# Rudrabha/Wav2Lip

Measured on NVIDIA H100. Metric: 96x96 face-crops/sec (B=128, T=5, mel 80x16), higher is better.
Workload: dtype f16

## Files before the change

### include/w2l.h

```cpp
#ifndef W2L_H_
#define W2L_H_

#include <stdint.h>

#ifdef __cplusplus
extern "C" {
#endif

#define W2L_ABI_VERSION 1

#define W2L_OK        0
#define W2L_EINVAL   -1
#define W2L_ENODEV   -2
#define W2L_ECUDA    -3
#define W2L_ENOMEM   -4
#define W2L_ESTATE   -5

#define W2L_NET_GENERATOR 0
#define W2L_NET_SYNCNET   1
#define W2L_NET_DISC      2
#define W2L_NET_S3FD      3

#define W2L_BLOCK_CONV_BN_RELU   0
#define W2L_BLOCK_CONVT_BN_RELU  1
// ... 75 lines not shown

int w2l_debug_layer_output(w2l_ctx* ctx, int net, int layer, float* y_dev, int* n, int* c, int* h, int* w,
                           void* stream);

int w2l_melspectrogram(w2l_ctx* ctx, const float* wav_dev, int64_t n_samples, float* mel_dev, void* stream);
int w2l_melspectrogram_host(w2l_ctx* ctx, const float* wav_host, int64_t n_samples, float* mel_host);
int64_t w2l_mel_num_frames(int64_t n_samples);

int64_t w2l_mel_num_chunks(int64_t n_frames, double fps);
int w2l_mel_chunks(w2l_ctx* ctx, const float* mel_dev, int64_t n_frames, double fps, float* chunks_dev,
                   int64_t n_chunks, void* stream);

int w2l_set_debug(w2l_ctx* ctx, int keep_all_layer_outputs);
int w2l_mel_basis_host(float* out_host);

#define W2L_KFAM_IGEMM        0
#define W2L_KFAM_PATCH        1
#define W2L_KFAM_CONVT_FUSED  2
typedef struct w2l_kernel_info {
    char    name[64];
    int32_t family;
    int32_t bn, bk, mt, head, bf16, x2, tma_epi, fold;
    int32_t m_tiles, n_tiles, grid;
} w2l_kernel_info;
int w2l_debug_kernel_table(int cap, w2l_kernel_info* out);
int w2l_debug_plan_kernels(w2l_ctx* ctx, int net, int cap, w2l_kernel_info* out);

#define W2L_TRAIN_WGRAD           1
#define W2L_TRAIN_ACCUMULATE      2
#define W2L_TRAIN_INPUT_GRAD      4
#define W2L_TRAIN_NO_STAT_UPDATE  8
int w2l_train_bind(w2l_ctx* ctx, int net, int n_tensors, const char* const* names, void* const* value_ptrs,
                   void* const* grad_ptrs, const int64_t* numels);

int w2l_train_forward(w2l_ctx* ctx, int net, const float* in0_dev, const float* in1_dev, float* out0_dev, float* out1_dev,
                      int B, int T, int flags, void* stream);

int w2l_train_backward(w2l_ctx* ctx, int net, const float* d0_dev, const float* d1_dev, float* dinput_dev, int flags,
                       void* stream);

int w2l_adam_step(w2l_ctx* ctx, int net, float lr, float beta1, float beta2, float eps, void* stream);

int w2l_wav2lip_train_step(w2l_ctx* ctx, const float* indiv_mels_dev, const float* x_dev, const float* mel_dev,
                           const float* gt_dev, int B, int T, float syncnet_wt, float lr, float* losses_dev, void* stream);
int w2l_train_last_output(w2l_ctx* ctx, float* out_dev, int64_t n, void* stream);
double w2l_train_flops(w2l_ctx* ctx, int net);
// ... 56 lines not shown
```

### wav2lip_b200/_lib.py

```python
from __future__ import annotations

import ctypes as C
import os
from typing import Optional

HERE = os.path.dirname(os.path.abspath(__file__))

W2L_OK, W2L_EINVAL, W2L_ENODEV, W2L_ECUDA, W2L_ENOMEM, W2L_ESTATE = 0, -1, -2, -3, -4, -5
NET_GENERATOR, NET_SYNCNET, NET_DISC, NET_S3FD = 0, 1, 2, 3
BLOCK_CONV_BN_RELU, BLOCK_CONVT_BN_RELU, BLOCK_CONV_LRELU, BLOCK_CONV_PLAIN, BLOCK_CONV_RELU = 0, 1, 2, 3, 4
PREC_F16, PREC_BF16, PREC_F32X = 0, 1, 2
TRAIN_WGRAD, TRAIN_ACCUMULATE, TRAIN_INPUT_GRAD, TRAIN_NO_STAT_UPDATE = 1, 2, 4, 8

EXPORTS = [
    "w2l_abi_version", "w2l_last_error", "w2l_net_num_layers", "w2l_net_layer_info",
    "w2l_create", "w2l_destroy", "w2l_load_weights",
    "w2l_generator_forward", "w2l_generator_forward_host", "w2l_generator_forward_u8", "w2l_generator_forward_u8_host",
    "w2l_generator_submit_host", "w2l_generator_submit_u8_host", "w2l_host_wait",
    "w2l_syncnet_forward", "w2l_syncnet_forward_frames", "w2l_cosine_bce_loss", "w2l_l1_loss", "w2l_disc_forward",
    "w2l_conv_block_forward", "w2l_debug_layer_output",
    "w2l_melspectrogram", "w2l_melspectrogram_host", "w2l_mel_num_frames", "w2l_mel_num_chunks", "w2l_mel_chunks",
    "w2l_set_debug", "w2l_mel_basis_host", "w2l_launch_count", "w2l_device_bytes", "w2l_profile_plan",
    "w2l_f16_overflow",
    "w2l_crop_resize_u8", "w2l_paste_u8", "w2l_lipsync_frames_u8", "w2l_s3fd_out_dims", "w2l_s3fd_forward",
    "w2l_train_bind", "w2l_train_forward", "w2l_train_backward", "w2l_adam_step", "w2l_wav2lip_train_step",
    "w2l_train_last_output", "w2l_train_flops", "w2l_comm_unique_id", "w2l_comm_init", "w2l_conv_block_train", "w2l_train_profile",
    "w2l_debug_kernel_table", "w2l_debug_plan_kernels", "w2l_debug_train_blocks", "w2l_debug_train_tensor",
]
KFAM_IGEMM, KFAM_PATCH, KFAM_CONVT_FUSED = 0, 1, 2
WG_PLAIN, WG_STRIDED, WG_TRANSPOSED, WG_SWAP, WG_FOLDED = 0, 1, 2, 3, 4
TAPE_X, TAPE_Z, TAPE_Y, TAPE_DY, TAPE_DZ, TAPE_DU, TAPE_DX, TAPE_DX_ADD, TAPE_STATS = range(9)


class W2LError(RuntimeError):
    pass


class LayerInfo(C.Structure):
    _fields_ = [("name", C.c_char * 64), ("kind", C.c_int32), ("cin", C.c_int32), ("cout", C.c_int32),
                ("kh", C.c_int32), ("kw", C.c_int32), ("sh", C.c_int32), ("sw", C.c_int32),
                ("ph", C.c_int32), ("pw", C.c_int32), ("out_pad", C.c_int32), ("residual", C.c_int32), ("cout_real", C.c_int32)]


class KernelInfo(C.Structure):
    _fields_ = [("name", C.c_char * 64), ("family", C.c_int32), ("bn", C.c_int32), ("bk", C.c_int32), ("mt", C.c_int32),
                ("head", C.c_int32), ("bf16", C.c_int32), ("x2", C.c_int32), ("tma_epi", C.c_int32), ("fold", C.c_int32),
                ("m_tiles", C.c_int32), ("n_tiles", C.c_int32), ("grid", C.c_int32)]

    def as_dict(self) -> dict:
        d = {f: getattr(self, f) for f, _ in self._fields_}
        d["name"] = self.name.decode()
        return d


class TrainBlockInfo(C.Structure):
    _fields_ = ([("name", C.c_char * 64)]
                + [(f, C.c_int32) for f in (
                    "layer", "kind", "cin", "cout", "kh", "kw", "sh", "sw", "ph", "pw", "out_pad", "residual",
                    "n", "h_in", "w_in", "h_out", "w_out", "lane", "has_dx", "has_dx_add", "has_du", "has_wgrad",
                    "wg_bn", "wg_form", "wg_ntaps", "wg_tg", "wg_ngroups", "wg_p", "wg_bw", "wg_bh", "wg_bnb",
                    "wg_chunks", "wg_m_tiles", "wg_n_tiles", "wg_splits", "wg_grid", "n_fwd", "n_dgrad")]
                + [("fwd", KernelInfo * 4), ("dgrad", KernelInfo * 4)])

    def as_dict(self) -> dict:
        d = {f: getattr(self, f) for f, _ in self._fields_ if f not in ("name", "fwd", "dgrad")}
        d["name"] = self.name.decode()
        d["fwd"] = [self.fwd[i].as_dict() for i in range(self.n_fwd)]
        d["dgrad"] = [self.dgrad[i].as_dict() for i in range(self.n_dgrad)]
        return d

# ... 209 lines not shown
```

### wav2lip_b200/csrc/conv_igemm.cuh

```cuda
#pragma once

#include <cuda.h>
#include <cuda_bf16.h>
#include <cuda_fp16.h>
#include <stdint.h>

#include "wgmma.cuh"

namespace w2l {

constexpr int kTileM = 128;
constexpr int kMaxTaps = 49;
constexpr int kMaxSteps = 3 * kMaxTaps;
constexpr int kSmemExtra = 2048;
constexpr int kSmemMax = 227 * 1024;
constexpr int kSmemBudget = kSmemMax - kSmemExtra - 2 * xbuf_bytes<32>();

enum : int { ACT_NONE = 0, ACT_RELU = 1, ACT_LRELU = 2 };

struct EpiParams {
    int Wout, Hout, N;
    int act;
    int out_f32;
    void* out;
    long long out_sn, out_sy, out_sx;
    const void* res;
    long long res_sn, res_sy, res_sx;
    const float* scale;
    const float* shift;
    const float* head_w;
    const float* head_b;
    int x2;
    int out_lo_off, res_lo_off;
    float* head_out;
    unsigned char* head_out_u8;
    int head_B, head_T;
};

struct alignas(64) ConvParams {
    CUtensorMap tmA;
    CUtensorMap tmB;
    CUtensorMap tmO;
    CUtensorMap tmR;
    int tma_epi;
    unsigned epi_box_bytes;
    int tiles_x, tiles_y, tiles_n, n_tiles;
    int bw, bh, bn;
    int sx, sy;
    int ntaps, kc_per_tap;
    unsigned stage_tx_bytes;
    EpiParams ep;
    int a_lo_off;
    signed char dx[kMaxSteps];
    signed char dy[kMaxSteps];
    unsigned char a_lo[kMaxSteps];
    unsigned char b_slab[kMaxSteps];
};

__device__ __forceinline__ uint32_t smem_u32(const void* p) {
    return static_cast<uint32_t>(__cvta_generic_to_shared(p));
}
__device__ __forceinline__ void mbar_init(uint32_t bar, uint32_t count) {
    asm volatile("mbarrier.init.shared::cta.b64 [%0], %1;" ::"r"(bar), "r"(count) : "memory");
}
__device__ __forceinline__ void mbar_arrive(uint32_t bar) {
    asm volatile("mbarrier.arrive.shared::cta.b64 _, [%0];" ::"r"(bar) : "memory");
// ... 10 lines not shown
        "@p bra W2L_DONE_%=;\n\t"
        "bra W2L_WAIT_%=;\n\t"
        "W2L_DONE_%=:\n\t"
        "}" ::"r"(bar), "r"(parity)
        : "memory");
}
__device__ __forceinline__ void fence_barrier_init() {
    asm volatile("fence.mbarrier_init.release.cluster;" ::: "memory");
}
__device__ __forceinline__ void tma_prefetch_desc(const void* desc) {
    asm volatile("prefetch.tensormap [%0];" ::"l"(reinterpret_cast<uint64_t>(desc)) : "memory");
}
__device__ __forceinline__ void tma_load_4d(uint32_t dst, const void* desc, uint32_t bar, int c0, int c1, int c2,
                                            int c3) {
    asm volatile(
        "cp.async.bulk.tensor.4d.shared::cluster.global.mbarrier::complete_tx::bytes [%0], [%1, {%3, %4, %5, %6}], [%2];"
        ::"r"(dst), "l"(reinterpret_cast<uint64_t>(desc)), "r"(bar), "r"(c0), "r"(c1), "r"(c2), "r"(c3)
        : "memory");
}
__device__ __forceinline__ void tma_load_3d(uint32_t dst, const void* desc, uint32_t bar, int c0, int c1, int c2) {
    asm volatile(
        "cp.async.bulk.tensor.3d.shared::cluster.global.mbarrier::complete_tx::bytes [%0], [%1, {%3, %4, %5}], [%2];"
        ::"r"(dst), "l"(reinterpret_cast<uint64_t>(desc)), "r"(bar), "r"(c0), "r"(c1), "r"(c2)
        : "memory");
}
__device__ __forceinline__ void pdl_launch_dependents() { asm volatile("griddepcontrol.launch_dependents;" ::: "memory"); }
__device__ __forceinline__ void pdl_wait() { asm volatile("griddepcontrol.wait;" ::: "memory"); }

template <int BK>
__device__ __forceinline__ uint64_t make_kmajor_desc(uint32_t saddr) {
    return wg_desc(saddr, 16, 8 * BK * 2, BK * 2);
}

template <int BN, int BK, bool kBF16>
__device__ __forceinline__ void wg_mma_tile(float (&acc)[2][BN / 2], uint32_t a, uint32_t sbo_a, uint32_t b, bool accumulate) {
#pragma unroll
    for (int k = 0; k < BK / 16; ++k) {
        const uint64_t bd = make_kmajor_desc<BK>(b + 32u * k);
        const uint32_t on = (accumulate || k > 0) ? 1u : 0u;
        wgmma_m64k16<BN, kBF16>(acc[0], wg_desc(a + 32u * k, 16, sbo_a, BK * 2), bd, on, 0);
        wgmma_m64k16<BN, kBF16>(acc[1], wg_desc(a + 8u * sbo_a + 32u * k, 16, sbo_a, BK * 2), bd, on, 0);
    }
}

template <int BN, int BK, int MT = 1>
struct ConvCfg {
// ... 152 lines not shown
    static_assert(!kHead || BN == 32, "fused head expects the 32-channel output block");
    static_assert(MT == 1 || MT == 2, "one or two M tiles per unit");

    extern __shared__ uint8_t smem_raw[];
    const uint32_t smem_raw_u32 = smem_u32(smem_raw);
    const uint32_t smem_base = (smem_raw_u32 + 1023u) & ~1023u;
    const uint32_t grp_base = smem_base + Cfg::kRingBytes;
    const uint32_t bar_base = grp_base + 2 * Cfg::kGrpBytes;
    auto full_bar = [&](int s) { return bar_base + 8u * s; };
    auto empty_bar = [&](int s) { return bar_base + 8u * (kStages + s); };
    auto res_bar = [&](int g) { return bar_base + 8u * (2 * kStages + g); };

    const int warp = threadIdx.x >> 5;
    const int lane = threadIdx.x & 31;

    if (warp == 0 && lane == 0) {
        tma_prefetch_desc(&p.tmA);
        tma_prefetch_desc(&p.tmB);
        if (p.tma_epi) {
            tma_prefetch_desc(&p.tmO);
            tma_prefetch_desc(&p.tmR);
        }
    }
    if (warp == 1 && lane == 0) {
        for (int s = 0; s < kStages; ++s) {
            mbar_init(full_bar(s), 1);
            mbar_init(empty_bar(s), 4 * MT);
        }
        for (int g = 0; g < 2; ++g) mbar_init(res_bar(g), 1);
        fence_barrier_init();
    }
    __syncthreads();
    pdl_wait();

    const int m_tiles = p.tiles_x * p.tiles_y * p.tiles_n;
    const int m_units = (m_tiles + MT - 1) / MT;
    const int total_tiles = m_units * p.n_tiles;
    const int k_steps = p.ntaps * p.kc_per_tap;

    if (warp < 4) {
        setmaxnreg_dec<kProducerRegs>();
        if (warp == 0 && lane == 0) {
            int stage = 0;
            uint32_t phase = 0;
            for (int tile = blockIdx.x; tile < total_tiles; tile += gridDim.x) {
                const int nt = tile % p.n_tiles;
                const int mu = tile / p.n_tiles;
                int x_in0[MT], y_in0[MT], n0[MT];
#pragma unroll
                for (int mt = 0; mt < MT; ++mt) {
                    const int m = mu * MT + mt;
                    const int tx = m % p.tiles_x;
                    const int ty = (m / p.tiles_x) % p.tiles_y;
                    const int tn = m / (p.tiles_x * p.tiles_y);
                    x_in0[mt] = tx * p.bw * p.sx;
                    y_in0[mt] = ty * p.bh * p.sy;
                    n0[mt] = tn * p.bn;
                }
                for (int t = 0; t < p.ntaps; ++t) {
                    for (int kc = 0; kc < p.kc_per_tap; ++kc) {
                        mbar_wait(empty_bar(stage), phase ^ 1u);
                        const uint32_t a_dst = smem_base + stage * Cfg::kStageBytes;
                        const uint32_t b_dst = a_dst + Cfg::kABytes;
                        mbar_arrive_expect_tx(full_bar(stage), p.stage_tx_bytes);
#pragma unroll
                        for (int mt = 0; mt < MT; ++mt)
                            tma_load_4d(a_dst + mt * Cfg::kATile, &p.tmA, full_bar(stage), kc * BK + (p.a_lo[t] ? p.a_lo_off : 0),
                                        x_in0[mt] + p.dx[t], y_in0[mt] + p.dy[t], n0[mt]);
                        tma_load_3d(b_dst, &p.tmB, full_bar(stage), kc * BK, nt * BN, p.b_slab[t]);
                        if (++stage == kStages) { stage = 0; phase ^= 1u; }
                    }
                }
            }
        }
    } else {
        setmaxnreg_inc<kConsumerRegs>();
        const int g = (warp - 4) >> 2;
        const int q = (warp - 4) & 3;
        const int mt = MT == 2 ? g : 0;
        constexpr int kItStride = MT == 2 ? 1 : 2;
        const int it0 = MT == 2 ? 0 : g;
        const int rows_valid = p.bw * p.bh * p.bn;
        const uint32_t bar_id = 1 + g;
        const uint32_t my_turn = 3 + g, their_turn = 3 + (g ^ 1);
        const uint32_t grp = grp_base + g * Cfg::kGrpBytes;
        float acc[2][BN / 2];
        auto mainloop = [&](int s0, bool hand_off) {
            int stage = s0 % kStages;
            uint32_t phase = static_cast<uint32_t>(s0 / kStages) & 1u;
            int prev = -1;
            for (int ks = 0; ks < k_steps; ++ks) {
                mbar_wait(full_bar(stage), phase);
                const uint32_t a_addr = smem_base + stage * Cfg::kStageBytes + mt * Cfg::kATile;
                wg_fence();
                wg_mma_tile<BN, BK, kBF16>(acc, a_addr, 8 * BK * 2, smem_base + stage * Cfg::kStageBytes + Cfg::kABytes, ks > 0);
                wg_commit();
                wg_wait<1>();
                if (prev >= 0 && lane == 0) mbar_arrive(empty_bar(prev));
                prev = stage;
                if (++stage == kStages) { stage = 0; phase ^= 1u; }
            }
            if (hand_off) named_bar_arrive(their_turn, 256);
            wg_wait<0>();
            wg_fence_regs<BN / 2>(acc[0]);
            wg_fence_regs<BN / 2>(acc[1]);
            if (prev >= 0 && lane == 0) mbar_arrive(empty_bar(prev));
        };
        auto for_each_tile = [&](auto&& epilogue) {
            for (int it = it0;; it += kItStride) {
                const int tile = blockIdx.x + it * static_cast<int>(gridDim.x);
                if (tile >= total_tiles) break;
                if (MT == 1 && it > 0) named_bar_sync(my_turn, 256);
                mainloop(it * k_steps, MT == 1 && tile + static_cast<int>(gridDim.x) < total_tiles);
                epilogue(tile, tile + kItStride * static_cast<int>(gridDim.x) < total_tiles);
            }
        };
        auto tile_origin = [&](int tile_, int* nt_, int* x0_, int* y0_, int* n0_) {
            *nt_ = tile_ % p.n_tiles;
            const int m_ = (tile_ / p.n_tiles) * MT + mt;
            *x0_ = (m_ % p.tiles_x) * p.bw;
            *y0_ = ((m_ / p.tiles_x) % p.tiles_y) * p.bh;
            *n0_ = (m_ / (p.tiles_x * p.tiles_y)) * p.bn;
        };
        if (!kHead && p.tma_epi) {
            constexpr int EW = Cfg::kEW;
            constexpr int kPasses = Cfg::kPasses;
            constexpr uint32_t kRowB = EW * 2;
            constexpr uint32_t kSwz = (kRowB == 128) ? 7u : (kRowB == 64) ? 3u : 1u;
            const bool leader = (q == 0 && lane == 0);
            const bool has_res = p.ep.res != nullptr;
            const EpiParams& e = p.ep;
            auto fetch_res = [&](int tile_) {
                int nt_, x0_, y0_, n0_;
                tile_origin(tile_, &nt_, &x0_, &y0_, &n0_);
                mbar_arrive_expect_tx(res_bar(g), kPasses * p.epi_box_bytes);
#pragma unroll
                for (int ps = 0; ps < kPasses; ++ps)
                    tma_load_4d(grp + ps * Cfg::kBoxBytes, &p.tmR, res_bar(g), nt_ * BN + ps * EW, x0_, y0_, n0_);
            };
            if (has_res && leader) {
                const int first = blockIdx.x + it0 * static_cast<int>(gridDim.x);
                if (first < total_tiles) fetch_res(first);
            }
            uint32_t rphase = 0;
            for_each_tile([&](int tile, bool more) {
                int nt, x0, y0, n0;
                tile_origin(tile, &nt, &x0, &y0, &n0);
                if (has_res) {
                    mbar_wait(res_bar(g), rphase);
                    rphase ^= 1u;
                }
                const float* const scale = e.scale + nt * BN;
                const float* const shift = e.shift + nt * BN;
#pragma unroll
                for (int j = 0; j < BN / 8; ++j) {
                    const int c = 8 * j + 2 * (lane & 3);
                    const float2 sc = __ldg(reinterpret_cast<const float2*>(scale + c));
                    const float2 sh = __ldg(reinterpret_cast<const float2*>(shift + c));
                    const uint32_t box = grp + (8 * j / EW) * Cfg::kBoxBytes;
#pragma unroll
                    for (int h = 0; h < 2; ++h) {
#pragma unroll
                        for (int r8 = 0; r8 < 2; ++r8) {
                            const int row = 64 * h + 16 * q + (lane >> 2) + 8 * r8;
                            float f0 = fmaf(acc[h][4 * j + 2 * r8], sc.x, sh.x);
// ... 10 lines not shown
                            if (e.act == ACT_RELU) {
                                f0 = fmaxf(f0, 0.0f);
                                f1 = fmaxf(f1, 0.0f);
                            } else if (e.act == ACT_LRELU) {
                                f0 = f0 > 0.0f ? f0 : 0.01f * f0;
                                f1 = f1 > 0.0f ? f1 : 0.01f * f1;
                            }
                            const uint32_t o = pack2<kBF16>(f0, f1, row < rows_valid);
                            asm volatile("st.shared.b32 [%0], %1;" ::"r"(a), "r"(o) : "memory");
                        }
                    }
                }
                asm volatile("fence.proxy.async.shared::cta;" ::: "memory");
                named_bar_sync(bar_id, 128);
                if (leader) {
#pragma unroll
                    for (int ps = 0; ps < kPasses; ++ps)
                        asm volatile("cp.async.bulk.tensor.4d.global.shared::cta.bulk_group [%0, {%2, %3, %4, %5}], [%1];"
                                     ::"l"(reinterpret_cast<uint64_t>(&p.tmO)), "r"(grp + ps * Cfg::kBoxBytes), "r"(nt * BN + ps * EW),
                                       "r"(x0), "r"(y0), "r"(n0)
                                     : "memory");
                    asm volatile("cp.async.bulk.commit_group;" ::: "memory");
                    asm volatile("cp.async.bulk.wait_group.read 0;" ::: "memory");
                    if (has_res && more) fetch_res(tile + kItStride * static_cast<int>(gridDim.x));
                }
                if (has_res)
                    __syncwarp();
                else
                    named_bar_sync(bar_id, 128);
            });
            if (leader) asm volatile("cp.async.bulk.wait_group 0;" ::: "memory");
        } else {
            const int row = q * 32 + lane;
            const int px = row % p.bw;
            const int py = (row / p.bw) % p.bh;
            const int pn = row / (p.bw * p.bh);
            float* const xb = reinterpret_cast<float*>(smem_raw + (grp - smem_raw_u32));
            for_each_tile([&](int tile, bool) {
                int nt, x0, y0, n0;
                tile_origin(tile, &nt, &x0, &y0, &n0);
                const int x = x0 + px, y = y0 + py, n = n0 + pn;
                const bool valid = (row < rows_valid) && (x < p.ep.Wout) && (y < p.ep.Hout) && (n < p.ep.N);
                epilogue_tile<BN, kBF16, kHead>(p.ep, acc, xb, bar_id, valid, n, y, x, nt);
            });
        }
    }
}

}
```

### wav2lip_b200/csrc/host_launch.cuh

```cuda
#pragma once

typedef void (*ConvKernelFn)(const ConvParams);
struct ConvKernelEntry { int BN, BK; bool bf16, head; ConvKernelFn fn; int smem; uint64_t attr_set; int mt; int threads; };

#define W2L_CONV_ENTRY(BN_, BK_)                                                                                                        \
    {BN_, BK_, false, false, conv_igemm_kernel<BN_, BK_, false, false>, ConvCfg<BN_, BK_>::kSmemBytes, 0, 1, ConvCfg<BN_, BK_>::kThreads}, \
    {BN_, BK_, true, false, conv_igemm_kernel<BN_, BK_, true, false>, ConvCfg<BN_, BK_>::kSmemBytes, 0, 1, ConvCfg<BN_, BK_>::kThreads}
#define W2L_CONV_ENTRY_MT2(BN_, BK_)                                                                                                    \
    {BN_, BK_, false, false, conv_igemm_kernel<BN_, BK_, false, false, 2>, ConvCfg<BN_, BK_, 2>::kSmemBytes, 0, 2, ConvCfg<BN_, BK_, 2>::kThreads}, \
    {BN_, BK_, true, false, conv_igemm_kernel<BN_, BK_, true, false, 2>, ConvCfg<BN_, BK_, 2>::kSmemBytes, 0, 2, ConvCfg<BN_, BK_, 2>::kThreads}

static ConvKernelEntry g_conv_kernels[] = {
    W2L_CONV_ENTRY(16, 16), W2L_CONV_ENTRY(16, 32), W2L_CONV_ENTRY(16, 64),
    W2L_CONV_ENTRY(32, 16), W2L_CONV_ENTRY(32, 32), W2L_CONV_ENTRY(32, 64),
    W2L_CONV_ENTRY(64, 16), W2L_CONV_ENTRY(64, 32), W2L_CONV_ENTRY(64, 64),
    W2L_CONV_ENTRY(128, 16), W2L_CONV_ENTRY(128, 32), W2L_CONV_ENTRY(128, 64),
    W2L_CONV_ENTRY_MT2(64, 64), W2L_CONV_ENTRY_MT2(64, 32),
    {32, 16, false, true, conv_igemm_kernel<32, 16, false, true>, ConvCfg<32, 16>::kSmemBytes, 0, 1, ConvCfg<32, 16>::kThreads},
    {32, 16, true, true, conv_igemm_kernel<32, 16, true, true>, ConvCfg<32, 16>::kSmemBytes, 0, 1, ConvCfg<32, 16>::kThreads},
};

static ConvKernelEntry* find_conv_kernel(int BN, int BK, bool bf16, bool head, int mt = 1) {
    for (auto& e : g_conv_kernels)
        if (e.BN == BN && e.BK == BK && e.bf16 == bf16 && e.head == head && e.mt == mt) return &e;
    return nullptr;
}
// ... 12 lines not shown
};
static PatchKernelEntry* find_patch_kernel(int BN, int BK, bool bf16, bool head) {
    for (auto& e : g_patch_kernels)
        if (e.BN == BN && e.BK == BK && e.bf16 == bf16 && e.head == head) return &e;
    return nullptr;
}

typedef void (*CtKernelFn)(const ConvTParams);
struct CtKernelEntry { int BK; bool bf16; CtKernelFn fn; uint64_t attr_set; };
static CtKernelEntry g_ct_kernels[] = {
    {32, false, convt_fused_kernel<32, false>, 0}, {32, true, convt_fused_kernel<32, true>, 0},
};
constexpr int kCtSmemMax = 227 * 1024;

static int ensure_smem_attr(uint64_t* mask, int device, const void* fn, int bytes) {
    const uint64_t bit = 1ull << (device & 63);
    if (*mask & bit) return W2L_OK;
    CK(cudaFuncSetAttribute(fn, cudaFuncAttributeMaxDynamicSharedMemorySize, bytes));
    *mask |= bit;
    return W2L_OK;
}

template <typename P>
static cudaError_t launch_k(void (*fn)(const P), int grid, int block, size_t smem, cudaStream_t st, const P& p, bool pdl) {
    cudaLaunchConfig_t cfg;
    memset(&cfg, 0, sizeof(cfg));
    cfg.gridDim = dim3((unsigned)grid, 1, 1);
    cfg.blockDim = dim3((unsigned)block, 1, 1);
    cfg.dynamicSmemBytes = smem;
    cfg.stream = st;
    cudaLaunchAttribute at[1];
    at[0].id = cudaLaunchAttributeProgrammaticStreamSerialization;
    at[0].val.programmaticStreamSerializationAllowed = 1;
    cfg.attrs = at;
    cfg.numAttrs = pdl ? 1 : 0;
    return cudaLaunchKernelEx(&cfg, fn, p);
}

static void op_kernel_info(const w2l_ctx* ctx, const Op& op, w2l_kernel_info* k) {
    memset(k, 0, sizeof(*k));
    snprintf(k->name, sizeof(k->name), "%s", op.name.c_str());
    k->family = op.ctf ? W2L_KFAM_CONVT_FUSED : op.patch ? W2L_KFAM_PATCH : W2L_KFAM_IGEMM;
    k->bn = op.BN; k->bk = op.BK; k->mt = op.MT; k->head = op.head ? 1 : 0;
    k->bf16 = ctx->bf16 ? 1 : 0; k->x2 = ctx->x2 ? 1 : 0;
    k->tma_epi = (!op.ctf && !op.patch && op.cp.tma_epi) ? 1 : 0;
    k->fold = op.fold ? 1 : 0;
    k->m_tiles = op.m_tiles; k->n_tiles = op.n_tiles; k->grid = op.grid;
}

static int launch_conv(w2l_ctx* ctx, const Op& op, cudaStream_t st, bool pdl = true) {
    pdl = pdl && ctx->use_pdl;
    if (op.ctf) {
        CtKernelEntry* e = nullptr;
        for (auto& k : g_ct_kernels) if (k.BK == op.BK && k.bf16 == ctx->bf16) e = &k;
        if (!e) return fail(W2L_EINVAL, "no fused convT kernel for BK=%d", op.BK);
        CKR(ensure_smem_attr(&e->attr_set, ctx->device, (const void*)e->fn, kCtSmemMax));
        CK(launch_k(e->fn, op.grid, kCtThreads, op.dyn_smem, st, op.tp, pdl));
        ctx->launches++;
        return W2L_OK;
    }
    if (op.patch) {
        PatchKernelEntry* e = find_patch_kernel(op.BN, op.BK, ctx->bf16, op.head);
        if (!e) return fail(W2L_EINVAL, "no patch kernel for BN=%d BK=%d head=%d", op.BN, op.BK, (int)op.head);
        CKR(ensure_smem_attr(&e->attr_set, ctx->device, (const void*)e->fn, kSmemMax));
        CK(launch_k(e->fn, op.grid, kPatchThreads, op.dyn_smem, st, op.pp, pdl));
        ctx->launches++;
        return W2L_OK;
    }
    ConvKernelEntry* e = find_conv_kernel(op.BN, op.BK, ctx->bf16, op.head, op.MT);
    if (!e) return fail(W2L_EINVAL, "no conv kernel for BN=%d BK=%d head=%d MT=%d", op.BN, op.BK, (int)op.head, op.MT);
    CKR(ensure_smem_attr(&e->attr_set, ctx->device, (const void*)e->fn, e->smem));
    CK(launch_k(e->fn, op.grid, e->threads, (size_t)e->smem, st, op.cp, pdl));
    ctx->launches++;
    return W2L_OK;
}
```

### wav2lip_b200/csrc/host_ops.cuh

```cuda
#pragma once

static int pick_bk(int cin_pad) { return (cin_pad % 64 == 0) ? 64 : (cin_pad % 32 == 0) ? 32 : 16; }
static int round_up(int a, int b) { return (a + b - 1) / b * b; }

static void pick_box(int W, int H, int N, int sx, int sy, int* bw, int* bh, int* bn) {
    double best = 1e30;
    int b_w = 1, b_h = 1, b_n = 1;
    for (int w = 1; w <= std::min(W, kTileM); ++w) {
        if (w * sx > 256) break;
        for (int h = 1; h <= std::min(H, kTileM / w); ++h) {
            if (h * sy > 256) break;
            int n = std::min(kTileM / (w * h), std::max(N, 1));
            if (n < 1) continue;
            if (n > 256) n = 256;
            const double tiles = (double)((W + w - 1) / w) * ((H + h - 1) / h) * ((N + n - 1) / n);
            const double cost = tiles - 1e-6 * w - 1e-9 * h;
            if (cost < best) { best = cost; b_w = w; b_h = h; b_n = n; }
        }
    }
    *bw = b_w; *bh = b_h; *bn = b_n;
}

struct ConvArgs {
    std::string name;
// ... 177 lines not shown
    PatchGeom geom;
    if (patch_eligible(ctx, a, &geom)) return make_patch_op(ctx, pl, a, geom);
    Op op;
    op.type = OP_CONV;
    op.name = a.name + (w.fold ? " [fold]" : "");
    const int BK = pick_bk(w.cin_pad);
    int bw, bh, bn;
    pick_box(a.Wl, a.Hl, a.in.N, a.sx, a.sy, &bw, &bh, &bn);
    const int tiles_x = (a.Wl + bw - 1) / bw, tiles_y = (a.Hl + bh - 1) / bh, tiles_n = (a.in.N + bn - 1) / bn;
    const int m_tiles = tiles_x * tiles_y * tiles_n;
    int BN = 16;
    for (int cand : {128, 64, 32, 16})
        if (a.cout % cand == 0) { BN = cand; break; }
    if (a.head) BN = 32;
    else
        while (BN > 32 && m_tiles * (a.cout / BN) < ctx->num_sms && a.cout % (BN / 2) == 0) BN /= 2;
    if (w.cout_pad % BN != 0) return fail(W2L_EINVAL, "%s: cout_pad %d vs BN %d", a.name.c_str(), w.cout_pad, BN);
    op.BN = BN; op.BK = BK; op.head = a.head;
    const int n_tiles_ = a.cout / BN;
    if (ctx->use_mt2 && !a.head && find_conv_kernel(BN, BK, ctx->bf16, false, 2) &&
        (long long)((m_tiles + 1) / 2) * n_tiles_ >= 2LL * ctx->num_sms)
        op.MT = 2;
    if (op.MT == 2) op.name += " [2M]";

    ConvParams& p = op.cp;
    memset(&p, 0, sizeof(p));
    CKR(encode_act_map(ctx, &p.tmA, a.in, BK, bw * a.sx, bh * a.sy, bn, a.sx, a.sy, a.name.c_str()));
    CKR(encode_w_map(ctx, &p.tmB, w, BK, BN, a.name.c_str()));
    p.tiles_x = tiles_x; p.tiles_y = tiles_y; p.tiles_n = tiles_n; p.n_tiles = a.cout / BN;
    p.bw = bw; p.bh = bh; p.bn = bn;
    p.sx = a.sx; p.sy = a.sy;
    p.ntaps = w.ntaps; p.kc_per_tap = w.cin_pad / BK;
    p.stage_tx_bytes = (unsigned)(op.MT * bw * bh * bn * BK * 2 + BN * BK * 2);
    fill_epi(&p.ep, a);
    p.tma_epi = 0;
    if (ctx->use_tma_epi && !ctx->x2 && !a.head && !a.out.f32) {
        EncodeTiledFn enc = get_encode_fn();
        const int EW = BN < 64 ? BN : 64;
        const CUtensorMapDataType dt = ctx->bf16 ? CU_TENSOR_MAP_DATA_TYPE_BFLOAT16 : CU_TENSOR_MAP_DATA_TYPE_FLOAT16;
        const CUtensorMapSwizzle esw = EW == 64 ? CU_TENSOR_MAP_SWIZZLE_128B : EW == 32 ? CU_TENSOR_MAP_SWIZZLE_64B : CU_TENSOR_MAP_SWIZZLE_32B;
        cuuint64_t dims[4] = {(cuuint64_t)std::min(a.cout, a.out.C), (cuuint64_t)a.Wl, (cuuint64_t)a.Hl, (cuuint64_t)a.in.N};
        cuuint32_t box[4] = {(cuuint32_t)EW, (cuuint32_t)bw, (cuuint32_t)bh, (cuuint32_t)bn};
        cuuint32_t es[4] = {1, 1, 1, 1};
        cuuint64_t os[3] = {(cuuint64_t)p.ep.out_sx * 2, (cuuint64_t)p.ep.out_sy * 2, (cuuint64_t)p.ep.out_sn * 2};
        CUresult r = enc(&p.tmO, dt, 4, p.ep.out, dims, os, box, es, CU_TENSOR_MAP_INTERLEAVE_NONE, esw,
                         CU_TENSOR_MAP_L2_PROMOTION_L2_128B, CU_TENSOR_MAP_FLOAT_OOB_FILL_NONE);
        if (r != CUDA_SUCCESS) return fail(W2L_ECUDA, "%s: cuTensorMapEncodeTiled(out) failed with %d", a.name.c_str(), (int)r);
        if (a.res) {
            cuuint64_t rs[3] = {(cuuint64_t)p.ep.res_sx * 2, (cuuint64_t)p.ep.res_sy * 2, (cuuint64_t)p.ep.res_sn * 2};
            r = enc(&p.tmR, dt, 4, const_cast<void*>(p.ep.res), dims, rs, box, es, CU_TENSOR_MAP_INTERLEAVE_NONE, esw,
                    CU_TENSOR_MAP_L2_PROMOTION_L2_128B, CU_TENSOR_MAP_FLOAT_OOB_FILL_NONE);
            if (r != CUDA_SUCCESS) return fail(W2L_ECUDA, "%s: cuTensorMapEncodeTiled(res) failed with %d", a.name.c_str(), (int)r);
        } else {
            p.tmR = p.tmO;
        }
        p.tma_epi = 1;
        p.epi_box_bytes = (unsigned)(bw * bh * bn * EW * 2);
    }
    if (w.ntaps > kMaxTaps) return fail(W2L_EINVAL, "%s: too many taps", a.name.c_str());
    if (a.cout > a.out.C && !p.tma_epi && !a.head) return fail(W2L_ESTATE, "%s: %d computed channels for a %d-channel destination need the TMA-store epilogue", a.name.c_str(), a.cout, a.out.C);
    if (ctx->x2) {
        if (a.in.lo_off <= 0 || w.nslabs != 2 * w.ntaps) return fail(W2L_ESTATE, "%s: split-operand mode needs hi/lo planes", a.name.c_str());
        int k = 0;
        for (int t = 0; t < w.ntaps; ++t)
            for (int v = 0; v < 3; ++v, ++k) {
                p.dx[k] = w.dx[t]; p.dy[k] = w.dy[t];
                p.a_lo[k] = (v == 1) ? 1 : 0;
                p.b_slab[k] = (unsigned char)((v == 2) ? w.ntaps + t : t);
            }
        p.ntaps = 3 * w.ntaps;
        p.a_lo_off = a.in.lo_off;
    } else {
        for (int t = 0; t < w.ntaps; ++t) { p.dx[t] = w.dx[t]; p.dy[t] = w.dy[t]; p.a_lo[t] = 0; p.b_slab[t] = (unsigned char)t; }
    }
    const int total = ((m_tiles + op.MT - 1) / op.MT) * p.n_tiles;
    op.grid = std::min(total, ctx->num_sms);
    op.fold = w.fold; op.m_tiles = m_tiles; op.n_tiles = p.n_tiles;
    op.flops = 2.0 * a.macs_per_pixel * (double)a.Wl * a.Hl * a.in.N;
    pl->ops.push_back(op);
    return W2L_OK;
}

static int make_convt_fused_op(w2l_ctx* ctx, Plan* pl, const Layer& L, const LayerW& lw, const Act& in, const Act& out, int act = ACT_RELU) {
    EncodeTiledFn enc = get_encode_fn();
    if (!enc) return fail(W2L_ENODEV, "cuTensorMapEncodeTiled is not available");
    const PackedW& w = lw.ph.back();
    Op op;
    op.type = OP_CONV;
    op.name = L.name + " [fused 4-phase]";
    op.ctf = true;
    const int BK = 32;
    if (w.cin_pad % BK != 0) return fail(W2L_EINVAL, "%s: fused convT needs cin %% 32 == 0", L.name.c_str());
    op.BK = BK; op.BN = kCtBN;
    ConvTParams& t = op.tp;
    memset(&t, 0, sizeof(t));
    CKR(encode_act_map(ctx, &t.tmA, in, BK, kCtPW, kCtPH, 1, 1, 1, L.name.c_str()));
    {
        const CUtensorMapDataType dt = ctx->bf16 ? CU_TENSOR_MAP_DATA_TYPE_BFLOAT16 : CU_TENSOR_MAP_DATA_TYPE_FLOAT16;
        const CUtensorMapSwizzle sw = CU_TENSOR_MAP_SWIZZLE_64B;
// ... 99 lines not shown
```

### wav2lip_b200/csrc/host_types.h

```cpp
#pragma once

static thread_local std::string g_err;

static int fail(int code, const char* fmt, ...) {
    char buf[1024];
    va_list ap;
    va_start(ap, fmt);
    vsnprintf(buf, sizeof(buf), fmt, ap);
    va_end(ap);
    g_err = buf;
    return code;
}

#define CK(call)                                                                                         \
    do {                                                                                                 \
        cudaError_t e_ = (call);                                                                         \
        if (e_ != cudaSuccess)                                                                           \
            return fail(W2L_ECUDA, "%s failed: %s (%s:%d)", #call, cudaGetErrorString(e_), __FILE__, __LINE__); \
    } while (0)
#define CKR(expr)               \
    do {                        \
        int r_ = (expr);        \
        if (r_ != W2L_OK) return r_; \
    } while (0)
// ... 58 lines not shown
    std::vector<PackedW> ph;
    float* scale = nullptr;
    float* shift = nullptr;
    int n_scale = 0;
    bool gemm_convT = false;
    bool has_all_taps = false;
    bool loaded = false;
};

struct NetW {
    std::vector<LayerW> layers;
    float* head_w = nullptr;
    float* head_b = nullptr;
    bool loaded = false;
};

enum OpType { OP_CONV = 0, OP_INGEST = 1, OP_L2NORM = 2, OP_DISC_HEAD = 3, OP_MAXPOOL = 4, OP_CHAN_L2NORM = 5, OP_S3FD_EXPORT = 6 };

struct Op {
    int type = OP_CONV;
    std::string name;
    ConvParams cp;
    int BN = 0, BK = 0, MT = 1;
    bool head = false;
    int grid = 0;
    double flops = 0;
    bool patch = false;
    PatchParams pp;
    int dyn_smem = 0;
    bool ctf = false;
    ConvTParams tp;
    bool fold = false;
    int m_tiles = 0, n_tiles = 0;
    IngestParams ip;
    int ingest_src = 0;
    const void* aux_in = nullptr;
    int aux_rows = 0, aux_dim = 0;
    int aux_out = 0;
    int aux_pitch = 0, aux_lo = 0;
    const uint16_t* sp_in = nullptr; uint16_t* sp_out = nullptr; const float* sp_f32 = nullptr; const float* sp_w = nullptr;
    int sp_N = 0, sp_H = 0, sp_W = 0, sp_C = 0, sp_Cout = 0, sp_maxout = 0;
    int lane = 0;
    bool join_side = false;
};

struct Plan {
// ... 3 lines not shown
    std::vector<void*> allocs;
    size_t bytes = 0;
    std::map<int, Act> layer_out;
    long long last_used = 0;
    bool x2 = false;
    bool has_side = false;
};

struct FoldJob { const float* bias; int cout, reps, n_pad; float* scale; float* shift; };
struct TrainState;

struct w2l_ctx {
    std::vector<PackParams>* pack_rec = nullptr;
    std::vector<FoldJob>* fold_rec = nullptr;
    std::vector<PackFoldParams>* pack_fold_rec = nullptr;
    TrainState* train = nullptr;
    int device = 0;
    bool bf16 = false;
    bool x2 = false;
    int num_sms = 132;
    bool keep_all = false;
    bool use_patch = true;
    bool use_mt2 = true;
    bool use_aux_stream = true;
    bool use_wg_stream = true;
    bool use_tma_epi = true;
    bool use_fold_s2 = true;
    bool use_ctfused = true;
    bool use_fold = true;
    bool use_pdl = true;
    bool use_mel_v2 = true;
    NetW nets[4];
    float* s3fd_l2w[3] = {nullptr, nullptr, nullptr};
    std::map<std::string, std::unique_ptr<Plan>> plans;
    Plan* last_plan[4] = {nullptr, nullptr, nullptr, nullptr};
    std::vector<w2l_kernel_info> last_block_kernels;
    int64_t launches = 0;
    long long plan_clock = 0;
    size_t weight_bytes = 0;
    cudaStream_t stream = nullptr;
    cudaStream_t s_h2d = nullptr, s_d2h = nullptr;
    cudaStream_t s_side = nullptr;
    cudaEvent_t ev_fork = nullptr, ev_join = nullptr;
    bool use_side = true;
    cudaEvent_t ev_in[2] = {nullptr, nullptr}, ev_done[2] = {nullptr, nullptr}, ev_out[2] = {nullptr, nullptr};
    void* stage[6] = {nullptr, nullptr, nullptr, nullptr, nullptr, nullptr};
// ... 59 lines not shown
```

### wav2lip_b200/csrc/w2l_api.cu

```cuda
#include <cuda.h>
#include <cuda_runtime.h>

#include <algorithm>
#include <cmath>
#include <cstdarg>
#include <cstdio>
#include <cstdlib>
#include <cstring>
#include <dlfcn.h>
#include <functional>
#include <map>
#include <memory>
#include <string>
#include <vector>

#include "../../include/w2l.h"
#include "aux_kernels.cuh"
#include "conv_igemm.cuh"
#include "conv_patch.cuh"
#include "convt_fused.cuh"
#include "mel.cuh"
#include "netspec.h"
#include "resize.cuh"
#include "train_kernels.cuh"
// ... 56 lines not shown
    ctx->bf16 = precision == W2L_PREC_BF16;
    ctx->x2 = precision == W2L_PREC_F32X;
    ctx->num_sms = prop.multiProcessorCount;
    cudaError_t e = cudaStreamCreateWithFlags(&ctx->stream, cudaStreamNonBlocking);
    if (e == cudaSuccess) e = cudaStreamCreateWithFlags(&ctx->s_h2d, cudaStreamNonBlocking);
    if (e == cudaSuccess) e = cudaStreamCreateWithFlags(&ctx->s_d2h, cudaStreamNonBlocking);
    if (e == cudaSuccess) e = cudaStreamCreateWithFlags(&ctx->s_side, cudaStreamNonBlocking);
    if (e == cudaSuccess) e = cudaEventCreateWithFlags(&ctx->ev_fork, cudaEventDisableTiming);
    if (e == cudaSuccess) e = cudaEventCreateWithFlags(&ctx->ev_join, cudaEventDisableTiming);
    for (int i = 0; i < 2 && e == cudaSuccess; ++i) {
        e = cudaEventCreateWithFlags(&ctx->ev_in[i], cudaEventDisableTiming);
        if (e == cudaSuccess) e = cudaEventCreateWithFlags(&ctx->ev_done[i], cudaEventDisableTiming);
        if (e == cudaSuccess) e = cudaEventCreateWithFlags(&ctx->ev_out[i], cudaEventDisableTiming);
    }
    if (e != cudaSuccess) { w2l_destroy(ctx); return fail(W2L_ECUDA, "cudaStreamCreate: %s", cudaGetErrorString(e)); }
    int r = init_mel_tables(ctx);
    if (r != W2L_OK) { const std::string msg = g_err; w2l_destroy(ctx); g_err = msg; return r; }
    {
        auto enabled = [](const char* name) { const char* v = getenv(name); return !(v && v[0] == '1'); };
        ctx->use_patch = enabled("W2L_DISABLE_HALO");
        ctx->use_fold = enabled("W2L_DISABLE_FOLD");
        ctx->use_fold_s2 = enabled("W2L_DISABLE_FOLDS2");
        ctx->use_mt2 = enabled("W2L_DISABLE_MT2");
        ctx->use_wg_stream = enabled("W2L_DISABLE_WGSTREAM");
        ctx->use_aux_stream = enabled("W2L_DISABLE_AUXSTREAM");
        ctx->use_tma_epi = enabled("W2L_DISABLE_TMAEPI");
        ctx->use_ctfused = enabled("W2L_DISABLE_CTFUSED");
        ctx->use_side = enabled("W2L_DISABLE_SIDESTREAM");
        ctx->use_pdl = enabled("W2L_DISABLE_PDL");
        ctx->use_mel_v2 = enabled("W2L_DISABLE_MELV2");
        if (ctx->x2) {
            ctx->use_patch = ctx->use_fold = ctx->use_fold_s2 = ctx->use_ctfused = ctx->use_tma_epi = false;
        }
        if (ctx->use_fold) {
            Act probe;
            probe.base = (uint16_t*)ctx->mel_tw; probe.N = 2; probe.H = 16; probe.W = 16; probe.Cs = 8; probe.C = 64; probe.Wp = 24;
            CUtensorMap tm;
            if (encode_act_map(ctx, &tm, probe, 64, 8, 8, 2, 1, 1, "probe") != W2L_OK) { ctx->use_fold = false; g_err.clear(); }
        }
    }
    *out = ctx;
    return W2L_OK;
}

int w2l_destroy(w2l_ctx* ctx) {
    if (!ctx) return W2L_OK;
// ... 974 lines not shown
```

Before: 51300.

## Add 2-CTA cluster launch with TMA multicast of activation tiles in conv igemm

Conv implicit-GEMM layers with BN=128 and MT=1 can now launch as 2-CTA clusters. The two CTAs work on adjacent N tiles of the same M tile, and each loads half of the activation tile with multicast TMA into both CTAs' shared memory. The empty barriers now count consumers from both CTAs, and releases are signalled across the cluster with mapa. This is meant to halve global/L2 traffic for the activation operand, at the cost of cross-CTA synchronisation, cluster scheduling limits, and a grid sized by max active clusters.

```diff
diff --git a/include/w2l.h b/include/w2l.h
--- a/include/w2l.h
+++ b/include/w2l.h
@@ -121,6 +121,8 @@
     int32_t family;
     int32_t bn, bk, mt, head, bf16, x2, tma_epi, fold;
     int32_t m_tiles, n_tiles, grid;
+    int32_t cluster;
+    int32_t cluster_axis;
 } w2l_kernel_info;
 int w2l_debug_kernel_table(int cap, w2l_kernel_info* out);
 int w2l_debug_plan_kernels(w2l_ctx* ctx, int net, int cap, w2l_kernel_info* out);
diff --git a/wav2lip_b200/_lib.py b/wav2lip_b200/_lib.py
--- a/wav2lip_b200/_lib.py
+++ b/wav2lip_b200/_lib.py
@@ -45,7 +45,8 @@
 class KernelInfo(C.Structure):
     _fields_ = [("name", C.c_char * 64), ("family", C.c_int32), ("bn", C.c_int32), ("bk", C.c_int32), ("mt", C.c_int32),
                 ("head", C.c_int32), ("bf16", C.c_int32), ("x2", C.c_int32), ("tma_epi", C.c_int32), ("fold", C.c_int32),
-                ("m_tiles", C.c_int32), ("n_tiles", C.c_int32), ("grid", C.c_int32)]
+                ("m_tiles", C.c_int32), ("n_tiles", C.c_int32), ("grid", C.c_int32), ("cluster", C.c_int32),
+                ("cluster_axis", C.c_int32)]
 
     def as_dict(self) -> dict:
         d = {f: getattr(self, f) for f, _ in self._fields_}
diff --git a/wav2lip_b200/csrc/conv_igemm.cuh b/wav2lip_b200/csrc/conv_igemm.cuh
--- a/wav2lip_b200/csrc/conv_igemm.cuh
+++ b/wav2lip_b200/csrc/conv_igemm.cuh
@@ -42,6 +42,8 @@
     CUtensorMap tmB;
     CUtensorMap tmO;
     CUtensorMap tmR;
+    CUtensorMap tmH;
+    int hx, hy, hn;
     int tma_epi;
     unsigned epi_box_bytes;
     int tiles_x, tiles_y, tiles_n, n_tiles;
@@ -98,6 +100,36 @@
     asm volatile(
         "cp.async.bulk.tensor.3d.shared::cluster.global.mbarrier::complete_tx::bytes [%0], [%1, {%3, %4, %5}], [%2];"
         ::"r"(dst), "l"(reinterpret_cast<uint64_t>(desc)), "r"(bar), "r"(c0), "r"(c1), "r"(c2)
+        : "memory");
+}
+__device__ __forceinline__ void tma_load_4d_mc(uint32_t dst, const void* desc, uint32_t bar, uint16_t mask, int c0, int c1,
+                                               int c2, int c3) {
+    asm volatile(
+        "cp.async.bulk.tensor.4d.shared::cluster.global.mbarrier::complete_tx::bytes.multicast::cluster"
+        " [%0], [%1, {%4, %5, %6, %7}], [%2], %3;"
+        ::"r"(dst), "l"(reinterpret_cast<uint64_t>(desc)), "r"(bar), "h"(mask), "r"(c0), "r"(c1), "r"(c2), "r"(c3)
+        : "memory");
+}
+__device__ __forceinline__ uint32_t cluster_ctarank() {
+    uint32_t r;
+    asm volatile("mov.u32 %0, %%cluster_ctarank;" : "=r"(r));
+    return r;
+}
+__device__ __forceinline__ uint32_t cluster_nctarank() {
+    uint32_t r;
+    asm volatile("mov.u32 %0, %%cluster_nctarank;" : "=r"(r));
+    return r;
+}
+__device__ __forceinline__ void cluster_sync() {
+    asm volatile("barrier.cluster.arrive.release;\n\tbarrier.cluster.wait.acquire;" ::: "memory");
+}
+__device__ __forceinline__ void mbar_arrive_cluster(uint32_t bar, uint32_t cta) {
+    asm volatile(
+        "{\n\t"
+        ".reg .b32 ra;\n\t"
+        "mapa.shared::cluster.u32 ra, %0, %1;\n\t"
+        "mbarrier.arrive.shared::cluster.b64 _, [ra];\n\t"
+        "}" ::"r"(bar), "r"(cta)
         : "memory");
 }
 __device__ __forceinline__ void pdl_launch_dependents() { asm volatile("griddepcontrol.launch_dependents;" ::: "memory"); }
@@ -296,34 +328,44 @@
             tma_prefetch_desc(&p.tmR);
         }
     }
+    constexpr bool kCluster = MT == 1 && !kHead;
+    const int cl = kCluster ? static_cast<int>(cluster_nctarank()) : 1;
+    const int rank = kCluster ? static_cast<int>(cluster_ctarank()) : 0;
+
     if (warp == 1 && lane == 0) {
         for (int s = 0; s < kStages; ++s) {
             mbar_init(full_bar(s), 1);
-            mbar_init(empty_bar(s), 4 * MT);
+            mbar_init(empty_bar(s), 4 * MT * cl);
         }
         for (int g = 0; g < 2; ++g) mbar_init(res_bar(g), 1);
         fence_barrier_init();
     }
-    __syncthreads();
+    if (cl > 1)
+        cluster_sync();
+    else
+        __syncthreads();
     pdl_wait();
 
     const int m_tiles = p.tiles_x * p.tiles_y * p.tiles_n;
-    const int m_units = (m_tiles + MT - 1) / MT;
-    const int total_tiles = m_units * p.n_tiles;
+    const int n_units = p.n_tiles / cl;
+    const int total_units = ((m_tiles + MT - 1) / MT) * n_units;
+    const int cta0 = static_cast<int>(blockIdx.x) / cl;
+    const int ncta = static_cast<int>(gridDim.x) / cl;
     const int k_steps = p.ntaps * p.kc_per_tap;
+    auto unit_nt = [&](int u) { return (u % n_units) * cl + rank; };
+    auto unit_m = [&](int u, int mt_) { return (u / n_units) * MT + mt_; };
 
     if (warp < 4) {
         setmaxnreg_dec<kProducerRegs>();
         if (warp == 0 && lane == 0) {
             int stage = 0;
             uint32_t phase = 0;
-            for (int tile = blockIdx.x; tile < total_tiles; tile += gridDim.x) {
-                const int nt = tile % p.n_tiles;
-                const int mu = tile / p.n_tiles;
+            for (int u = cta0; u < total_units; u += ncta) {
+                const int nt = unit_nt(u);
                 int x_in0[MT], y_in0[MT], n0[MT];
 #pragma unroll
                 for (int mt = 0; mt < MT; ++mt) {
-                    const int m = mu * MT + mt;
+                    const int m = unit_m(u, mt);
                     const int tx = m % p.tiles_x;
                     const int ty = (m / p.tiles_x) % p.tiles_y;
                     const int tn = m / (p.tiles_x * p.tiles_y);
@@ -337,10 +379,16 @@
                         const uint32_t a_dst = smem_base + stage * Cfg::kStageBytes;
                         const uint32_t b_dst = a_dst + Cfg::kABytes;
                         mbar_arrive_expect_tx(full_bar(stage), p.stage_tx_bytes);
-#pragma unroll
-                        for (int mt = 0; mt < MT; ++mt)
-                            tma_load_4d(a_dst + mt * Cfg::kATile, &p.tmA, full_bar(stage), kc * BK + (p.a_lo[t] ? p.a_lo_off : 0),
-                                        x_in0[mt] + p.dx[t], y_in0[mt] + p.dy[t], n0[mt]);
+                        const int ca = kc * BK + (p.a_lo[t] ? p.a_lo_off : 0);
+                        if (cl == 2) {
+                            tma_load_4d_mc(a_dst + rank * (Cfg::kATile / 2), &p.tmH, full_bar(stage), 0x3, ca,
+                                           x_in0[0] + p.dx[t] + rank * p.hx, y_in0[0] + p.dy[t] + rank * p.hy, n0[0] + rank * p.hn);
+                        } else {
+#pragma unroll
+                            for (int mt = 0; mt < MT; ++mt)
+                                tma_load_4d(a_dst + mt * Cfg::kATile, &p.tmA, full_bar(stage), ca, x_in0[mt] + p.dx[t],
+                                            y_in0[mt] + p.dy[t], n0[mt]);
+                        }
                         tma_load_3d(b_dst, &p.tmB, full_bar(stage), kc * BK, nt * BN, p.b_slab[t]);
                         if (++stage == kStages) { stage = 0; phase ^= 1u; }
                     }
@@ -359,6 +407,14 @@
         const uint32_t my_turn = 3 + g, their_turn = 3 + (g ^ 1);
         const uint32_t grp = grp_base + g * Cfg::kGrpBytes;
         float acc[2][BN / 2];
+        auto release = [&](int s) {
+            if (cl == 1) {
+                mbar_arrive(empty_bar(s));
+            } else {
+                mbar_arrive_cluster(empty_bar(s), 0);
+                mbar_arrive_cluster(empty_bar(s), 1);
+            }
+        };
         auto mainloop = [&](int s0, bool hand_off) {
             int stage = s0 % kStages;
             uint32_t phase = static_cast<uint32_t>(s0 / kStages) & 1u;
@@ -370,7 +426,7 @@
                 wg_mma_tile<BN, BK, kBF16>(acc, a_addr, 8 * BK * 2, smem_base + stage * Cfg::kStageBytes + Cfg::kABytes, ks > 0);
                 wg_commit();
                 wg_wait<1>();
-                if (prev >= 0 && lane == 0) mbar_arrive(empty_bar(prev));
+                if (prev >= 0 && lane == 0) release(prev);
                 prev = stage;
                 if (++stage == kStages) { stage = 0; phase ^= 1u; }
             }
@@ -378,20 +434,20 @@
             wg_wait<0>();
             wg_fence_regs<BN / 2>(acc[0]);
             wg_fence_regs<BN / 2>(acc[1]);
-            if (prev >= 0 && lane == 0) mbar_arrive(empty_bar(prev));
+            if (prev >= 0 && lane == 0) release(prev);
         };
         auto for_each_tile = [&](auto&& epilogue) {
             for (int it = it0;; it += kItStride) {
-                const int tile = blockIdx.x + it * static_cast<int>(gridDim.x);
-                if (tile >= total_tiles) break;
+                const int u = cta0 + it * ncta;
+                if (u >= total_units) break;
                 if (MT == 1 && it > 0) named_bar_sync(my_turn, 256);
-                mainloop(it * k_steps, MT == 1 && tile + static_cast<int>(gridDim.x) < total_tiles);
-                epilogue(tile, tile + kItStride * static_cast<int>(gridDim.x) < total_tiles);
+                mainloop(it * k_steps, MT == 1 && u + ncta < total_units);
+                epilogue(u, u + kItStride * ncta < total_units);
             }
         };
-        auto tile_origin = [&](int tile_, int* nt_, int* x0_, int* y0_, int* n0_) {
-            *nt_ = tile_ % p.n_tiles;
-            const int m_ = (tile_ / p.n_tiles) * MT + mt;
+        auto tile_origin = [&](int u_, int* nt_, int* x0_, int* y0_, int* n0_) {
+            *nt_ = unit_nt(u_);
+            const int m_ = unit_m(u_, mt);
             *x0_ = (m_ % p.tiles_x) * p.bw;
             *y0_ = ((m_ / p.tiles_x) % p.tiles_y) * p.bh;
             *n0_ = (m_ / (p.tiles_x * p.tiles_y)) * p.bn;
@@ -413,8 +469,8 @@
                     tma_load_4d(grp + ps * Cfg::kBoxBytes, &p.tmR, res_bar(g), nt_ * BN + ps * EW, x0_, y0_, n0_);
             };
             if (has_res && leader) {
-                const int first = blockIdx.x + it0 * static_cast<int>(gridDim.x);
-                if (first < total_tiles) fetch_res(first);
+                const int first = cta0 + it0 * ncta;
+                if (first < total_units) fetch_res(first);
             }
             uint32_t rphase = 0;
             for_each_tile([&](int tile, bool more) {
@@ -471,7 +527,7 @@
                                      : "memory");
                     asm volatile("cp.async.bulk.commit_group;" ::: "memory");
                     asm volatile("cp.async.bulk.wait_group.read 0;" ::: "memory");
-                    if (has_res && more) fetch_res(tile + kItStride * static_cast<int>(gridDim.x));
+                    if (has_res && more) fetch_res(tile + kItStride * ncta);
                 }
                 if (has_res)
                     __syncwarp();
@@ -494,6 +550,7 @@
             });
         }
     }
-}
-
-}
+    if (cl > 1) cluster_sync();
+}
+
+}
diff --git a/wav2lip_b200/csrc/host_launch.cuh b/wav2lip_b200/csrc/host_launch.cuh
--- a/wav2lip_b200/csrc/host_launch.cuh
+++ b/wav2lip_b200/csrc/host_launch.cuh
@@ -1,7 +1,10 @@
 #pragma once
 
 typedef void (*ConvKernelFn)(const ConvParams);
-struct ConvKernelEntry { int BN, BK; bool bf16, head; ConvKernelFn fn; int smem; uint64_t attr_set; int mt; int threads; };
+struct ConvKernelEntry {
+    int BN, BK; bool bf16, head; ConvKernelFn fn; int smem; uint64_t attr_set; int mt; int threads;
+    int max_clusters2;
+};
 
 #define W2L_CONV_ENTRY(BN_, BK_)                                                                                                        \
     {BN_, BK_, false, false, conv_igemm_kernel<BN_, BK_, false, false>, ConvCfg<BN_, BK_>::kSmemBytes, 0, 1, ConvCfg<BN_, BK_>::kThreads}, \
@@ -60,19 +63,48 @@
 }
 
 template <typename P>
-static cudaError_t launch_k(void (*fn)(const P), int grid, int block, size_t smem, cudaStream_t st, const P& p, bool pdl) {
+static cudaError_t launch_k(void (*fn)(const P), int grid, int block, size_t smem, cudaStream_t st, const P& p, bool pdl,
+                            int cluster = 1) {
     cudaLaunchConfig_t cfg;
     memset(&cfg, 0, sizeof(cfg));
     cfg.gridDim = dim3((unsigned)grid, 1, 1);
     cfg.blockDim = dim3((unsigned)block, 1, 1);
     cfg.dynamicSmemBytes = smem;
     cfg.stream = st;
-    cudaLaunchAttribute at[1];
-    at[0].id = cudaLaunchAttributeProgrammaticStreamSerialization;
-    at[0].val.programmaticStreamSerializationAllowed = 1;
+    cudaLaunchAttribute at[2];
+    int n = 0;
+    if (pdl) {
+        at[n].id = cudaLaunchAttributeProgrammaticStreamSerialization;
+        at[n++].val.programmaticStreamSerializationAllowed = 1;
+    }
+    if (cluster > 1) {
+        at[n].id = cudaLaunchAttributeClusterDimension;
+        at[n++].val.clusterDim = {(unsigned)cluster, 1, 1};
+    }
     cfg.attrs = at;
-    cfg.numAttrs = pdl ? 1 : 0;
+    cfg.numAttrs = n;
     return cudaLaunchKernelEx(&cfg, fn, p);
+}
+
+static int conv_max_clusters2(w2l_ctx* ctx, ConvKernelEntry* e, int* out) {
+    if (e->max_clusters2 == 0) {
+        CKR(ensure_smem_attr(&e->attr_set, ctx->device, (const void*)e->fn, e->smem));
+        cudaLaunchConfig_t cfg;
+        memset(&cfg, 0, sizeof(cfg));
+        cfg.gridDim = dim3(2u * (unsigned)ctx->num_sms, 1, 1);
+        cfg.blockDim = dim3((unsigned)e->threads, 1, 1);
+        cfg.dynamicSmemBytes = (size_t)e->smem;
+        cudaLaunchAttribute at[1];
+        at[0].id = cudaLaunchAttributeClusterDimension;
+        at[0].val.clusterDim = {2u, 1, 1};
+        cfg.attrs = at;
+        cfg.numAttrs = 1;
+        int n = 0;
+        CK(cudaOccupancyMaxActiveClusters(&n, (const void*)e->fn, &cfg));
+        e->max_clusters2 = n > 0 ? n : -1;
+    }
+    *out = std::max(e->max_clusters2, 0);
+    return W2L_OK;
 }
 
 static void op_kernel_info(const w2l_ctx* ctx, const Op& op, w2l_kernel_info* k) {
@@ -84,6 +116,7 @@
     k->tma_epi = (!op.ctf && !op.patch && op.cp.tma_epi) ? 1 : 0;
     k->fold = op.fold ? 1 : 0;
     k->m_tiles = op.m_tiles; k->n_tiles = op.n_tiles; k->grid = op.grid;
+    k->cluster = op.cluster; k->cluster_axis = op.cluster > 1 ? 1 : 0;
 }
 
 static int launch_conv(w2l_ctx* ctx, const Op& op, cudaStream_t st, bool pdl = true) {
@@ -108,7 +141,7 @@
     ConvKernelEntry* e = find_conv_kernel(op.BN, op.BK, ctx->bf16, op.head, op.MT);
     if (!e) return fail(W2L_EINVAL, "no conv kernel for BN=%d BK=%d head=%d MT=%d", op.BN, op.BK, (int)op.head, op.MT);
     CKR(ensure_smem_attr(&e->attr_set, ctx->device, (const void*)e->fn, e->smem));
-    CK(launch_k(e->fn, op.grid, e->threads, (size_t)e->smem, st, op.cp, pdl));
+    CK(launch_k(e->fn, op.grid, e->threads, (size_t)e->smem, st, op.cp, pdl, op.cluster));
     ctx->launches++;
     return W2L_OK;
 }
diff --git a/wav2lip_b200/csrc/host_ops.cuh b/wav2lip_b200/csrc/host_ops.cuh
--- a/wav2lip_b200/csrc/host_ops.cuh
+++ b/wav2lip_b200/csrc/host_ops.cuh
@@ -223,6 +223,16 @@
         (long long)((m_tiles + 1) / 2) * n_tiles_ >= 2LL * ctx->num_sms)
         op.MT = 2;
     if (op.MT == 2) op.name += " [2M]";
+    const int k_steps = w.ntaps * (ctx->x2 ? 3 : 1) * (w.cin_pad / BK);
+    const int cl_units = m_tiles * (n_tiles_ / 2);
+    int max_c2 = 0;
+    bool cluster = false;
+    if (ctx->use_cluster && op.MT == 1 && !a.head && BN == 128 && n_tiles_ % 2 == 0 && bw * bh * bn == kTileM) {
+        ConvKernelEntry* e = find_conv_kernel(BN, BK, ctx->bf16, false, 1);
+        if (e) CKR(conv_max_clusters2(ctx, e, &max_c2));
+        cluster = max_c2 > 0 && cl_units >= max_c2 && (k_steps >= 64 || cl_units >= 16 * max_c2);
+    }
+    if (cluster) op.name += " [c2]";
 
     ConvParams& p = op.cp;
     memset(&p, 0, sizeof(p));
@@ -233,6 +243,13 @@
     p.sx = a.sx; p.sy = a.sy;
     p.ntaps = w.ntaps; p.kc_per_tap = w.cin_pad / BK;
     p.stage_tx_bytes = (unsigned)(op.MT * bw * bh * bn * BK * 2 + BN * BK * 2);
+    if (cluster) {
+        int hw = bw, hh = bh, hn = bn;
+        if (bn > 1) { hn = bn / 2; p.hn = hn; }
+        else if (bh > 1) { hh = bh / 2; p.hy = hh * a.sy; }
+        else { hw = bw / 2; p.hx = hw * a.sx; }
+        CKR(encode_act_map(ctx, &p.tmH, a.in, BK, hw * a.sx, hh * a.sy, hn, a.sx, a.sy, a.name.c_str()));
+    }
     fill_epi(&p.ep, a);
     p.tma_epi = 0;
     if (ctx->use_tma_epi && !ctx->x2 && !a.head && !a.out.f32) {
@@ -274,8 +291,13 @@
     } else {
         for (int t = 0; t < w.ntaps; ++t) { p.dx[t] = w.dx[t]; p.dy[t] = w.dy[t]; p.a_lo[t] = 0; p.b_slab[t] = (unsigned char)t; }
     }
-    const int total = ((m_tiles + op.MT - 1) / op.MT) * p.n_tiles;
-    op.grid = std::min(total, ctx->num_sms);
+    if (cluster) {
+        op.cluster = 2;
+        op.grid = 2 * std::min(cl_units, max_c2);
+    } else {
+        const int total = ((m_tiles + op.MT - 1) / op.MT) * p.n_tiles;
+        op.grid = std::min(total, ctx->num_sms);
+    }
     op.fold = w.fold; op.m_tiles = m_tiles; op.n_tiles = p.n_tiles;
     op.flops = 2.0 * a.macs_per_pixel * (double)a.Wl * a.Hl * a.in.N;
     pl->ops.push_back(op);
diff --git a/wav2lip_b200/csrc/host_types.h b/wav2lip_b200/csrc/host_types.h
--- a/wav2lip_b200/csrc/host_types.h
+++ b/wav2lip_b200/csrc/host_types.h
@@ -104,6 +104,7 @@
     std::string name;
     ConvParams cp;
     int BN = 0, BK = 0, MT = 1;
+    int cluster = 1;
     bool head = false;
     int grid = 0;
     double flops = 0;
@@ -153,6 +154,7 @@
     bool keep_all = false;
     bool use_patch = true;
     bool use_mt2 = true;
+    bool use_cluster = true;
     bool use_aux_stream = true;
     bool use_wg_stream = true;
     bool use_tma_epi = true;
diff --git a/wav2lip_b200/csrc/w2l_api.cu b/wav2lip_b200/csrc/w2l_api.cu
--- a/wav2lip_b200/csrc/w2l_api.cu
+++ b/wav2lip_b200/csrc/w2l_api.cu
@@ -102,6 +102,7 @@
         ctx->use_fold = enabled("W2L_DISABLE_FOLD");
         ctx->use_fold_s2 = enabled("W2L_DISABLE_FOLDS2");
         ctx->use_mt2 = enabled("W2L_DISABLE_MT2");
+        ctx->use_cluster = enabled("W2L_DISABLE_CLUSTER");
         ctx->use_wg_stream = enabled("W2L_DISABLE_WGSTREAM");
         ctx->use_aux_stream = enabled("W2L_DISABLE_AUXSTREAM");
         ctx->use_tma_epi = enabled("W2L_DISABLE_TMAEPI");
```

Result: faster. 52240, median of 6 (+1.8%).
